# AIM-SE/AC-TSR

Measured on AMD Instinct MI355X. Metric: user-sequences/sec fwd+bwd, AC-SASRec L=50 d=64, 1/2/4/8 MI355X, higher is better.
Workload: dtype f32; 1 GPU; ACSASRec full training step (spatial + adversarial calibrators, BASELINE configs[2]), synthetic 100000-item catalogue, B=512/GPU L=50 d=64 h=2 2 layers inner=256, CE loss, two-pass backward + Adam; global_batch=512, seq_len=50, hidden=64, heads=2, parallelism=dp1, launch=hipGraph replay per step, backward=two walks (reference protocol, trainer.py:672-686)

## Files before the change

ac_tsr_amd/csrc/acattn_bwd.hip:

```cpp
#include <stdlib.h>

#include "acattn_common.h"

int acattn_launch_bwd_general_dh16(const acattn_problem& p, const acattn_bwd_io& io, hipStream_t stream);
int acattn_launch_bwd_general_dh32(const acattn_problem& p, const acattn_bwd_io& io, hipStream_t stream);
int acattn_launch_bwd_general_dh64(const acattn_problem& p, const acattn_bwd_io& io, hipStream_t stream);
int acattn_launch_bwd_general_dh128(const acattn_problem& p, const acattn_bwd_io& io, hipStream_t stream);

int acattn_launch_bwd_fast(const acattn_problem& p, const acattn_bwd_io& io, hipStream_t stream);
int acattn_launch_bwd_stream(const acattn_problem& p, const acattn_bwd_io& io, hipStream_t stream);
int acattn_launch_bwd_onerow(const acattn_problem& p, const acattn_bwd_io& io, bool accumulate, hipStream_t stream);
int acattn_launch_bwd_long(const acattn_problem& p, const acattn_bwd_io& io, hipStream_t stream);

namespace {
thread_local int g_bwd_kernel = ACATTN_BWD_AUTO;
}
int acattn_bwd_kernel_choice(int which) {
  const int old = g_bwd_kernel;
  if (which >= ACATTN_BWD_AUTO && which <= ACATTN_BWD_LONG) g_bwd_kernel = which;
  return old;
}

bool acattn_bwd_onerow_applies(const acattn_problem& p, const acattn_bwd_io& io);

namespace {
bool onerow_split_applies(const acattn_problem& p, const acattn_bwd_io& io) {
  static const bool split = getenv("ACATTN_ONEROW_SPLIT") ? atoi(getenv("ACATTN_ONEROW_SPLIT")) != 0 : true;
  if (!(split && (io.d_attack_mask || io.d_penalty_part) && io.read_rows && io.n_read_rows == 1 && !io.active_qblocks && !io.attack_only && p.L <= 64))
    return false;
  const int dh = p.n_heads > 0 ? p.H / p.n_heads : 0;
  if (dh != 16 && dh != 32 && dh != 64) return false;
  acattn_bwd_io row_io = io;
  row_io.d_attack_mask = nullptr;
  row_io.d_penalty_part = nullptr;
  return acattn_bwd_onerow_applies(p, row_io);
}
}

bool acattn_bwd_gate_summed(const acattn_problem& p, const acattn_bwd_io& io) {
  if (g_bwd_kernel != ACATTN_BWD_AUTO || !io.dgate_logits) return false;
  return acattn_bwd_onerow_applies(p, io) || onerow_split_applies(p, io);
}

bool acattn_bwd_stream_pair_applies(const acattn_problem& p, const acattn_bwd_io& io);
bool acattn_bwd_pair_supported(const acattn_problem& p, const acattn_bwd_io& io) {
  const bool streaming = g_bwd_kernel == ACATTN_BWD_STREAM || (g_bwd_kernel == ACATTN_BWD_AUTO && p.L > 64);
  return streaming && acattn_bwd_stream_pair_applies(p, io);
}

int acattn_launch_bwd(const acattn_problem& p, const acattn_bwd_io& io, hipStream_t stream) {
  if (g_bwd_kernel == ACATTN_BWD_LONG || (g_bwd_kernel == ACATTN_BWD_AUTO && p.L > 208))
    return acattn_launch_bwd_long(p, io, stream);
  if (p.L > 208) {
    acattn_set_error("backward: the pinned kernel is built for L <= 208; L > 208 needs ACATTN_BWD_LONG or ACATTN_BWD_AUTO");
    return -1;
  }
  if ((io.dqa2 || io.dka2 || io.d_ctx_calibrated2 || io.d_penalty_part2) && !acattn_bwd_pair_supported(p, io)) {
    acattn_set_error("attention backward: a second cotangent set was given but this launch cannot evaluate it "
                     "(ask acattn_calibrated_attention_bwd_pair_supported first)");
    return -1;
  }
  if (io.dgate_summed && !acattn_bwd_gate_summed(p, io)) {
    acattn_set_error("attention backward: dgate_summed requested but this launch does not take the one-row form "
                     "(ask acattn_calibrated_attention_bwd_gate_summed first)");
    return -1;
  }
  const int which = g_bwd_kernel;
  if (which == ACATTN_BWD_AUTO) {
    const int rc_one = acattn_launch_bwd_onerow(p, io, false, stream);
    if (rc_one != -100) return rc_one;
    static const bool split = getenv("ACATTN_ONEROW_SPLIT") ? atoi(getenv("ACATTN_ONEROW_SPLIT")) != 0 : true;
    if (split && (io.d_attack_mask || io.d_penalty_part) && io.read_rows && io.n_read_rows == 1 && !io.active_qblocks && !io.attack_only && p.L <= 64) {
      acattn_bwd_io mask_io = io;
      mask_io.d_ctx_attacked = mask_io.d_ctx_calibrated = nullptr;
      mask_io.n_read_rows = 0;
      mask_io.attack_only = 1;
      const int rc_mask = acattn_launch_bwd_fast(p, mask_io, stream);
      if (rc_mask == 0) {
        acattn_bwd_io row_io = io;
        row_io.d_attack_mask = nullptr;
        row_io.d_penalty_part = nullptr;
        const int rc_row = acattn_launch_bwd_onerow(p, row_io, true, stream);
        if (rc_row != -100) return rc_row;
        acattn_set_error("attention backward: the mask-only launch ran but the one-row kernel does not cover this problem (read-row chain not computed)");
        return -1;
      }
      if (rc_mask != -100) return rc_mask;
    }
    if (io.dgate_summed) {
      acattn_set_error("attention backward: dgate_summed was accepted but no one-row form ran");
      return -1;
    }
  }
  static const bool short_stream = getenv("ACATTN_BWD_SHORT_STREAM") && atoi(getenv("ACATTN_BWD_SHORT_STREAM")) != 0;
  const bool short_rows = p.L <= 64 && !short_stream;
  if (which == ACATTN_BWD_AUTO && short_rows) {
    const int rc_fast = acattn_launch_bwd_fast(p, io, stream);
    if (rc_fast != -100) return rc_fast;
  }
  if (which == ACATTN_BWD_AUTO || which == ACATTN_BWD_STREAM) {
    const int rc_stream = acattn_launch_bwd_stream(p, io, stream);
    if (rc_stream != -100) return rc_stream;
  }
  const int rc_fast = acattn_launch_bwd_fast(p, io, stream);
  if (rc_fast != -100) return rc_fast;
  switch (p.H / p.n_heads) {
    case 16: return acattn_launch_bwd_general_dh16(p, io, stream);
    case 32: return acattn_launch_bwd_general_dh32(p, io, stream);
    case 64: return acattn_launch_bwd_general_dh64(p, io, stream);
    case 128: return acattn_launch_bwd_general_dh128(p, io, stream);
  }
  return -1;
}
```

ac_tsr_amd/csrc/acattn_bwd_stream.hip:

```cpp
#include <stdlib.h>

#include <algorithm>

#include "acattn_common.h"

namespace {

constexpr float kLog2e = 1.44269504088896340736f;
constexpr float kLn2 = 0.69314718055994530942f;

__device__ __forceinline__ float ex2(float x) { return __builtin_amdgcn_exp2f(x); }
__device__ __forceinline__ float and_bits(float x, int m) { return __uint_as_float(__float_as_uint(x) & (uint32_t)m); }
__device__ __forceinline__ float hsum(const f4 v) { return (v[0] + v[1]) + (v[2] + v[3]); }
__device__ __forceinline__ float row16_sum(float v) {
  v += __builtin_bit_cast(float, __builtin_amdgcn_update_dpp(0, __builtin_bit_cast(int, v), 0xB1, 0xF, 0xF, false));
  v += __builtin_bit_cast(float, __builtin_amdgcn_update_dpp(0, __builtin_bit_cast(int, v), 0x4E, 0xF, 0xF, false));
  v += __builtin_bit_cast(float, __builtin_amdgcn_update_dpp(0, __builtin_bit_cast(int, v), 0x141, 0xF, 0xF, false));
  v += __builtin_bit_cast(float, __builtin_amdgcn_update_dpp(0, __builtin_bit_cast(int, v), 0x140, 0xF, 0xF, false));
  return v;
}

#ifndef ACATTN_BWD_ONE_WAVE_DH
#define ACATTN_BWD_ONE_WAVE_DH 64
#endif
// ... 842 lines not shown
  } while (0)
#else
#define OR_STAMP(k)
#endif

template <int DH, bool ACC, bool SLICED>
__global__ void __launch_bounds__(64) acattn_bwd_onerow_kernel(const acattn_problem P, const acattn_bwd_io IO) {
#ifdef ACATTN_ONEROW_STAMPS
  unsigned long long cyc_[8] = {}, last_ = 0;
#endif
  OR_STAMP(-1);
  constexpr int D4 = DH / 4;
  __shared__ __attribute__((aligned(16))) float vec[8][DH];
  __shared__ __attribute__((aligned(16))) float col[4][256];
  const int L = P.L, H = P.H, nh = P.n_heads;
  const int nT = (L + 15) >> 4;
  const bool causal = P.causal != 0;
  int b, h;
  decode_block(blockIdx.x, P.B, nh, b, h);
  const int lane = threadIdx.x;
  const size_t rowbase = (size_t)b * L, bh = (size_t)b * nh + h;
  const int hoff = h * DH;
  const int i = min(max((int)IO.read_rows[b], 0), L - 1);
  const KeyFlags F = load_key_flags(P.key_valid, rowbase, L, nT, lane);
  const Consts K = make_consts(P, DH);

  for (int d = lane; d < DH; d += 64) {
    const size_t o = (rowbase + i) * H + hoff + d;
    vec[0][d] = P.q[o];
    vec[1][d] = P.qa[o];
    vec[2][d] = IO.d_ctx_attacked ? IO.d_ctx_attacked[o] : 0.f;
    vec[3][d] = IO.d_ctx_calibrated ? IO.d_ctx_calibrated[o] : 0.f;
    vec[4][d] = P.w_order[DH + d] * -kLog2e;
    vec[5][d] = P.w_dist[DH + d];
    vec[6][d] = P.w_order[d];
    vec[7][d] = P.w_dist[d];
  }
  __syncthreads();
  OR_STAMP(0);
  RowScalars R;
  {
    float ao = 0.f, adv = 0.f;
#pragma unroll
    for (int d = 0; d < DH; ++d) {
      ao += vec[0][d] * vec[6][d];
      adv += vec[0][d] * vec[7][d];
    }
    R.ao2 = -kLog2e * (ao + P.b_order[0]);
    R.ad = adv + P.b_dist[0];
  }
  const bool dead = causal ? F.first_valid > i : !F.any_valid;
  {
    const float sh = dead ? ACATTN_MASK_FILL : 0.f;
    const float* sp = IO.row_stats + (bh * L + i) * ACATTN_NSTAT;
    R.lx2 = (sp[0] - sh) * kLog2e;
    R.ly2 = (sp[1] - sh) * kLog2e;
    R.lu2 = (sp[2] - sh) * kLog2e;
    R.lv2 = (sp[3] - sh) * kLog2e;
    R.lw2 = (sp[4] - sh) * kLog2e;
  }
  R.i = i;
  R.rng_row = (uint32_t)(bh * L + i);
  const bool order_select = !causal || dead;

  constexpr bool sliced = SLICED;
  constexpr int N4 = SLICED ? D4 / 4 : D4;
  const int kgrp = sliced ? (lane & 15) : lane;
  const int slice = sliced ? (lane >> 4) : 0;
  const int d_lo = slice * N4;
  const float lead = slice == 0 ? 1.0f : 0.0f;
  const int t = kgrp >> 2, g = kgrp & 3, j0 = 4 * kgrp;
  f4 aS = {0.f, 0.f, 0.f, 0.f}, aM = aS, aP = aS, aW = aS, co4 = aS, cd4 = aS;
  if constexpr (SLICED) {
#pragma unroll
    for (int r = 0; r < 4; ++r) {
      const size_t o = (rowbase + min(j0 + r, L - 1)) * H + hoff;
#pragma unroll
      for (int k4 = 0; k4 < N4; ++k4) {
        const int d4 = d_lo + k4;
        const f4 kv = *(const f4*)(P.k + o + 4 * d4), kav = *(const f4*)(P.ka + o + 4 * d4), vv = *(const f4*)(P.v + o + 4 * d4);
        const f4 q4 = *(const f4*)(&vec[0][4 * d4]), qa4 = *(const f4*)(&vec[1][4 * d4]);
        const f4 ga4 = *(const f4*)(&vec[2][4 * d4]), gc4 = *(const f4*)(&vec[3][4 * d4]);
        const f4 wo4 = *(const f4*)(&vec[4][4 * d4]), wd4 = *(const f4*)(&vec[5][4 * d4]);
        aS[r] += hsum(kv * q4);
        aM[r] += hsum(kav * qa4);
        aP[r] += hsum(vv * ga4);
        aW[r] += hsum(vv * gc4);
        co4[r] += hsum(kv * wo4);
        cd4[r] += hsum(kv * wd4);
      }
    }
  } else {
    size_t o4[4];
#pragma unroll
    for (int r = 0; r < 4; ++r) o4[r] = (rowbase + min(j0 + r, L - 1)) * H + hoff;
#pragma unroll 2
    for (int k4 = 0; k4 < N4; ++k4) {
      const f4 q4 = *(const f4*)(&vec[0][4 * k4]), qa4 = *(const f4*)(&vec[1][4 * k4]);
      const f4 ga4 = *(const f4*)(&vec[2][4 * k4]), gc4 = *(const f4*)(&vec[3][4 * k4]);
      const f4 wo4 = *(const f4*)(&vec[4][4 * k4]), wd4 = *(const f4*)(&vec[5][4 * k4]);
      f4 kv[4], kav[4], vv[4];
#pragma unroll
      for (int r = 0; r < 4; ++r) {
        kv[r] = *(const f4*)(P.k + o4[r] + 4 * k4);
        kav[r] = *(const f4*)(P.ka + o4[r] + 4 * k4);
        vv[r] = *(const f4*)(P.v + o4[r] + 4 * k4);
      }
#pragma unroll
      for (int r = 0; r < 4; ++r) {
        aS[r] += hsum(kv[r] * q4);
        aM[r] += hsum(kav[r] * qa4);
        aP[r] += hsum(vv[r] * ga4);
        aW[r] += hsum(vv[r] * gc4);
        co4[r] += hsum(kv[r] * wo4);
        cd4[r] += hsum(kv[r] * wd4);
      }
    }
    __builtin_amdgcn_sched_barrier(0);
  }
  if (sliced) {
#pragma unroll
    for (int r = 0; r < 4; ++r) {
      aS[r] = quad_sum(aS[r]);
      aM[r] = quad_sum(aM[r]);
      aP[r] = quad_sum(aP[r]);
      aW[r] = quad_sum(aW[r]);
      co4[r] = quad_sum(co4[r]);
      cd4[r] = quad_sum(cd4[r]);
    }
  }
  OR_STAMP(1);
  const f4 gl = load_seg(P.gate_logits + (rowbase + i) * L, j0, L, true);
  uint32_t eb4, ab4;
  tile_bits(F, t, g, i, L, causal, true, dead, eb4, ab4);
  if (j0 >= 16 * nT) eb4 = 0u;
  Tile T;
  tile_elementwise(R, K, aS, aM, aP, aW, co4, cd4, gl, t, g, eb4, ab4, order_select, T);

  const float da = wave_sum(lead * hsum(T.Ap * T.dAp)), dc = wave_sum(lead * hsum(T.Aw * T.dAw));
  const f4 dw = T.Aw * (T.dAw - dc);
  const f4 dac = (1.0f - T.gt) * dw;
  const float r1 = wave_sum(lead * hsum(T.Ac * dac));
  const f4 du = T.Ap * (T.dAp - da), dv = T.Ac * (dac - r1);
  f4 dP = T.gt * dw + dv * T.ex1 + du * T.M;
  f4 dM = du * (T.P - T.nz) - dv * (T.P * T.ex1);
#pragma unroll
  for (int r = 0; r < 4; ++r) {
    dP[r] = keep_and(dP[r] * K.keep_scale, T.ka, r);
    dM[r] = keep_and(dM[r] * K.keep_scale, T.km, r);
  }
  const float sP = wave_sum(lead * hsum(T.Pt * dP)), sM = wave_sum(lead * hsum(T.Mt * dM));
  f4 dS, dSa, dgl, d_o, d_d;
  float dsc;
  tile_backward(T, K, da, dc, r1, sP, sM, f4{0.f, 0.f, 0.f, 0.f}, i, j0, dS, dSa, dgl, d_o, d_d, dsc);
  const float da_o = wave_sum(lead * hsum(d_o)), da_d = wave_sum(lead * hsum(d_d)), dsc_sum = wave_sum(lead * dsc);
  if (slice == 0) {
    *(f4*)(&col[0][j0]) = dS;
    *(f4*)(&col[1][j0]) = dSa;
    *(f4*)(&col[2][j0]) = d_o;
    *(f4*)(&col[3][j0]) = d_d;
  }

  OR_STAMP(2);
  if constexpr (SLICED) {
#pragma unroll
    for (int r = 0; r < 4; ++r) {
      const int j = j0 + r;
      if (j < L) {
        const size_t o = (rowbase + j) * H + hoff;
#pragma unroll
        for (int k4 = 0; k4 < N4; ++k4) {
          const int d4 = d_lo + k4;
          const f4 q4 = *(const f4*)(&vec[0][4 * d4]), qa4 = *(const f4*)(&vec[1][4 * d4]);
          const f4 ga4 = *(const f4*)(&vec[2][4 * d4]), gc4 = *(const f4*)(&vec[3][4 * d4]);
          const f4 wo_hi = *(const f4*)(P.w_order + DH + 4 * d4), wd_hi = *(const f4*)(P.w_dist + DH + 4 * d4);
          *(f4*)(IO.dk + o + 4 * d4) = q4 * dS[r] + wo_hi * d_o[r] + wd_hi * d_d[r];
          if (ACC)
            *(f4*)(IO.dka + o + 4 * d4) += qa4 * dSa[r];
          else
            *(f4*)(IO.dka + o + 4 * d4) = qa4 * dSa[r];
          *(f4*)(IO.dv + o + 4 * d4) = ga4 * T.Ap[r] + gc4 * T.Aw[r];
        }
      }
    }
  } else {
#pragma unroll 2
    for (int k4 = 0; k4 < N4; ++k4) {
      const f4 q4 = *(const f4*)(&vec[0][4 * k4]), qa4 = *(const f4*)(&vec[1][4 * k4]);
      const f4 ga4 = *(const f4*)(&vec[2][4 * k4]), gc4 = *(const f4*)(&vec[3][4 * k4]);
      const f4 wo_hi = *(const f4*)(P.w_order + DH + 4 * k4), wd_hi = *(const f4*)(P.w_dist + DH + 4 * k4);
#pragma unroll
      for (int r = 0; r < 4; ++r) {
        const int j = j0 + r;
        if (j < L) {
          const size_t o = (rowbase + j) * H + hoff;
          *(f4*)(IO.dk + o + 4 * k4) = q4 * dS[r] + wo_hi * d_o[r] + wd_hi * d_d[r];
          if (ACC)
            *(f4*)(IO.dka + o + 4 * k4) += qa4 * dSa[r];
          else
            *(f4*)(IO.dka + o + 4 * k4) = qa4 * dSa[r];
          *(f4*)(IO.dv + o + 4 * k4) = ga4 * T.Ap[r] + gc4 * T.Aw[r];
        }
      }
    }
    __builtin_amdgcn_sched_barrier(0);
  }
  OR_STAMP(3);
  if (IO.dgate_logits && IO.dgate_summed) {
    if (slice == 0) {
      float* grow = IO.dgate_logits + ((size_t)b * L + i) * L;
#pragma unroll
      for (int r = 0; r < 4; ++r)
        if (j0 + r < L) atomicAdd(grow + j0 + r, dgl[r]);
    }
  } else if (IO.dgate_logits) {
    float* gbase = IO.dgate_logits + bh * (size_t)L * L;
    for (int row = 0; row < L; ++row) {
      if (row == i) continue;
      for (int j = lane; j < L; j += 64) gbase[(size_t)row * L + j] = 0.f;
    }
    if (slice == 0) store_seg(gbase + (size_t)i * L, j0, L, true, dgl);
  }
  __syncthreads();
  OR_STAMP(4);

  const int stride_w = IO.part_stride ? IO.part_stride : 2 * DH, stride_s = IO.part_stride ? IO.part_stride : 4;
  constexpr int PARTS = DH <= 32 ? 64 / DH : 1;
  constexpr int NCH = DH > 64 ? DH / 64 : 1;
#pragma unroll 1
  for (int ch = 0; ch < NCH; ++ch) {
    const int d = (DH > 64 ? lane : lane % DH) + 64 * ch, part = DH > 64 ? 0 : lane / DH;
    float sq = 0.f, sqa = 0.f, so = 0.f, sd = 0.f;
    constexpr int UJ = 8;
    for (int jb = part; jb < L; jb += PARTS * UJ) {
      float kv[UJ], kav[UJ];
#pragma unroll
      for (int u = 0; u < UJ; ++u) {
        const int j = min(jb + u * PARTS, L - 1);
        const size_t o = (rowbase + j) * H + hoff + d;
        kv[u] = P.k[o];
        kav[u] = P.ka[o];
      }
#pragma unroll
      for (int u = 0; u < UJ; ++u) {
        const int j = jb + u * PARTS;
        const float w = j < L ? 1.0f : 0.0f;
        const int jc = min(j, L - 1);
        sq += w * col[0][jc] * kv[u];
        sqa += w * col[1][jc] * kav[u];
        so += w * col[2][jc] * kv[u];
        sd += w * col[3][jc] * kv[u];
      }
    }
#pragma unroll
    for (int off = DH; off < 64; off <<= 1) {
      sq += __shfl_xor(sq, off);
      sqa += __shfl_xor(sqa, off);
      so += __shfl_xor(so, off);
      sd += __shfl_xor(sd, off);
    }
    if (ch == 0) {
      constexpr int LPR = DH / 4, RPI = 64 / LPR;
      const f4 z4 = {0.f, 0.f, 0.f, 0.f};
      for (int row = lane / LPR; row < L; row += RPI) {
        if (row == i) continue;
        const size_t o = (rowbase + row) * H + hoff + 4 * (lane % LPR);
        *(f4*)(IO.dq + o) = z4;
        if (!ACC) *(f4*)(IO.dqa + o) = z4;
      }
    }
    if (part == 0) {
      const size_t o = (rowbase + i) * H + hoff + d;
      IO.dq[o] = sq + da_o * vec[6][d] + da_d * vec[7][d];
      if (ACC) IO.dqa[o] += sqa;
      else IO.dqa[o] = sqa;
    }
    if (part != 0) continue;
    IO.dw_order_part[bh * stride_w + d] = da_o * vec[0][d];
    IO.dw_dist_part[bh * stride_w + d] = da_d * vec[0][d];
    IO.dw_order_part[bh * stride_w + DH + d] = so;
    IO.dw_dist_part[bh * stride_w + DH + d] = sd;
  }
  if (lane == 0) {
    float* sm = IO.dsmall_part + bh * stride_s;
    sm[0] = da_o;
    sm[1] = da_d;
    sm[2] = dsc_sum;
    sm[3] = 0.f;
  }
  OR_STAMP(5);
#ifdef ACATTN_ONEROW_STAMPS
  if (lane == 0 && blockIdx.x < 2048)
    for (int k = 0; k < 8; ++k) g_onerow_stamps[blockIdx.x * 8 + k] = cyc_[k];
#endif
}

#ifdef ACATTN_ONEROW_STAMPS
extern "C" int acattn_debug_onerow_stamps(unsigned long long* host, int n_words) {
  return (int)hipMemcpyFromSymbol(host, HIP_SYMBOL(g_onerow_stamps), (size_t)n_words * 8);
}
#endif

template <int DH>
int launch_onerow(const acattn_problem& p, const acattn_bwd_io& io, bool accumulate, hipStream_t stream) {
  const dim3 grid(p.B * p.n_heads), block(64);
  if (io.dgate_logits && io.dgate_summed) {
    const int rc = acattn_launch_zero(io.dgate_logits, (size_t)p.B * p.L * p.L, stream);
    if (rc) return rc;
  }
  if (p.L <= 64) {
    if (accumulate)
      hipLaunchKernelGGL((acattn_bwd_onerow_kernel<DH, true, true>), grid, block, 0, stream, p, io);
    else
      hipLaunchKernelGGL((acattn_bwd_onerow_kernel<DH, false, true>), grid, block, 0, stream, p, io);
  } else if (accumulate) {
    hipLaunchKernelGGL((acattn_bwd_onerow_kernel<DH, true, false>), grid, block, 0, stream, p, io);
  } else {
    hipLaunchKernelGGL((acattn_bwd_onerow_kernel<DH, false, false>), grid, block, 0, stream, p, io);
  }
  return (int)hipGetLastError();
}

template <int DH>
int launch_stream(const acattn_problem& p, const acattn_bwd_io& io, float* ws, hipStream_t stream) {
  const int nT = (p.L + 15) / 16, dh = DH;
  const size_t rows = (size_t)p.B * p.n_heads;
  if (!io.attack_only) {
    int rc = 0;
    auto zero = [&](float* ptr, size_t n) { if (!rc) rc = acattn_launch_zero(ptr, n, stream); };
    if (io.part_stride) {
      float* lo = std::min(io.dw_order_part, std::min(io.dw_dist_part, io.dsmall_part));
      zero(lo, rows * io.part_stride);
    } else {
      zero(io.dw_order_part, rows * 2 * dh);
      zero(io.dw_dist_part, rows * 2 * dh);
      zero(io.dsmall_part, rows * 4);
    }
    if (rc) return rc;
  }
  const dim3 grid(p.B * p.n_heads * nT), block(64);
  static const bool no_dca_form = getenv("ACATTN_BWD_DCA_ALWAYS") ? atoi(getenv("ACATTN_BWD_DCA_ALWAYS")) == 0 : true;
  if (io.d_ctx_attacked || !no_dca_form) {
    hipLaunchKernelGGL((acattn_bwd_row_kernel<DH, true>), grid, block, 0, stream, p, io, ws);
    hipLaunchKernelGGL((acattn_bwd_key_kernel<DH, true>), grid, block, 0, stream, p, io, (const float*)ws);
  } else if (io.dqa2) {
    hipLaunchKernelGGL((acattn_bwd_row_kernel<DH, false, true>), grid, block, 0, stream, p, io, ws);
    hipLaunchKernelGGL((acattn_bwd_key_kernel<DH, false, true>), grid, block, 0, stream, p, io, (const float*)ws);
  } else {
    hipLaunchKernelGGL((acattn_bwd_row_kernel<DH, false>), grid, block, 0, stream, p, io, ws);
    hipLaunchKernelGGL((acattn_bwd_key_kernel<DH, false>), grid, block, 0, stream, p, io, (const float*)ws);
  }
  return (int)hipGetLastError();
}

}

int64_t acattn_bwd_stream_ws_bytes(const acattn_problem& p) { return (int64_t)p.B * p.n_heads * p.L * NSC * sizeof(float); }

bool acattn_bwd_onerow_applies(const acattn_problem& p, const acattn_bwd_io& io) {
  static const bool enabled = getenv("ACATTN_ONEROW") ? atoi(getenv("ACATTN_ONEROW")) != 0 : true;
  const int dh = p.n_heads > 0 ? p.H / p.n_heads : 0;
  return enabled && io.read_rows && io.n_read_rows == 1 && !io.active_qblocks && !io.d_attack_mask && !io.d_penalty_part && !io.attack_only &&
         p.L <= 208 && (int64_t)p.B * p.n_heads * p.L * p.L < (1LL << 30) && (int64_t)p.B * p.L * p.H < (1LL << 30) &&
         p.mask_mode == ACATTN_MASK_STRUCTURED && p.rng_mode == ACATTN_RNG_COUNTER && p.w_order && p.w_dist &&
         p.adversarial && p.combine_option == ACATTN_COMBINE_GATE && p.two_level && (dh == 16 || dh == 32 || dh == 64 || dh == 128);
}

int acattn_launch_bwd_onerow(const acattn_problem& p, const acattn_bwd_io& io, bool accumulate, hipStream_t stream) {
  if (!acattn_bwd_onerow_applies(p, io)) return -100;
  switch (p.H / p.n_heads) {
    case 16: return launch_onerow<16>(p, io, accumulate, stream);
    case 32: return launch_onerow<32>(p, io, accumulate, stream);
    case 64: return launch_onerow<64>(p, io, accumulate, stream);
    case 128: return launch_onerow<128>(p, io, accumulate, stream);
  }
  return -100;
}

bool acattn_bwd_stream_pair_applies(const acattn_problem& p, const acattn_bwd_io& io) {
  const int dh = p.n_heads > 0 ? p.H / p.n_heads : 0;
  return io.workspace && p.L <= 208 && (int64_t)p.B * p.n_heads * p.L * p.L < (1LL << 30) && (int64_t)p.B * p.L * p.H < (1LL << 30) &&
         p.mask_mode == ACATTN_MASK_STRUCTURED && p.rng_mode == ACATTN_RNG_COUNTER && p.w_order && p.w_dist && p.adversarial &&
         p.combine_option == ACATTN_COMBINE_GATE && p.two_level && (dh == 16 || dh == 32 || dh == 64) && !io.d_ctx_attacked &&
         !io.attack_only && !io.read_rows && !io.active_qblocks && io.dqa2 && io.dka2 &&
         (io.d_ctx_calibrated2 || io.d_penalty_part2);
}

int acattn_launch_bwd_stream(const acattn_problem& p, const acattn_bwd_io& io, hipStream_t stream) {
  const bool ok = io.workspace && p.L <= 208 && (int64_t)p.B * p.n_heads * p.L * p.L < (1LL << 30) &&
                  (int64_t)p.B * p.L * p.H < (1LL << 30) && p.mask_mode == ACATTN_MASK_STRUCTURED &&
                  p.rng_mode == ACATTN_RNG_COUNTER && p.w_order && p.w_dist && p.adversarial &&
                  p.combine_option == ACATTN_COMBINE_GATE && p.two_level;
  if (!ok) return -100;
  float* ws = (float*)io.workspace;
  switch (p.H / p.n_heads) {
    case 16: return launch_stream<16>(p, io, ws, stream);
    case 32: return launch_stream<32>(p, io, ws, stream);
    case 64: return launch_stream<64>(p, io, ws, stream);
    case 128: return launch_stream<128>(p, io, ws, stream);
  }
  return -100;
}
```

Measured before the change: 531,100 user-sequences/sec.

## Add dedicated attack-only attention backward kernel and fold gate zeroing into it

Adds a specialised backward kernel for the attack-mask/penalty-only pass. It runs one block per (batch, head) with one wave per 16-row query block, and builds dK from LDS slot partials without atomics. The same kernel also zeroes the summed gate-logit gradient buffer, so the one-row kernel can skip its separate zero-fill launch. This is meant to replace the generic fast kernel on this path and remove one launch. In exchange it adds sizeable LDS per block and a fallback turn-taking path when there are too few slots.

Result: faster. 537,200 user-sequences/sec, median of 6 (+1.2%).

```diff
diff --git a/ac_tsr_amd/csrc/acattn_bwd.hip b/ac_tsr_amd/csrc/acattn_bwd.hip
--- a/ac_tsr_amd/csrc/acattn_bwd.hip
+++ b/ac_tsr_amd/csrc/acattn_bwd.hip
@@ -9,7 +9,8 @@
 
 int acattn_launch_bwd_fast(const acattn_problem& p, const acattn_bwd_io& io, hipStream_t stream);
 int acattn_launch_bwd_stream(const acattn_problem& p, const acattn_bwd_io& io, hipStream_t stream);
-int acattn_launch_bwd_onerow(const acattn_problem& p, const acattn_bwd_io& io, bool accumulate, hipStream_t stream);
+int acattn_launch_bwd_attack(const acattn_problem& p, const acattn_bwd_io& io, hipStream_t stream, float* gate_zero = nullptr);
+int acattn_launch_bwd_onerow(const acattn_problem& p, const acattn_bwd_io& io, bool accumulate, hipStream_t stream, bool gate_zeroed = false);
 int acattn_launch_bwd_long(const acattn_problem& p, const acattn_bwd_io& io, hipStream_t stream);
 
 namespace {
@@ -24,6 +25,10 @@
 bool acattn_bwd_onerow_applies(const acattn_problem& p, const acattn_bwd_io& io);
 
 namespace {
+bool attack_kernel_enabled() {
+  static const bool on = getenv("ACATTN_BWD_ATTACK") ? atoi(getenv("ACATTN_BWD_ATTACK")) != 0 : true;
+  return on;
+}
 bool onerow_split_applies(const acattn_problem& p, const acattn_bwd_io& io) {
   static const bool split = getenv("ACATTN_ONEROW_SPLIT") ? atoi(getenv("ACATTN_ONEROW_SPLIT")) != 0 : true;
   if (!(split && (io.d_attack_mask || io.d_penalty_part) && io.read_rows && io.n_read_rows == 1 && !io.active_qblocks && !io.attack_only && p.L <= 64))
@@ -75,12 +80,15 @@
       mask_io.d_ctx_attacked = mask_io.d_ctx_calibrated = nullptr;
       mask_io.n_read_rows = 0;
       mask_io.attack_only = 1;
-      const int rc_mask = acattn_launch_bwd_fast(p, mask_io, stream);
+      float* gate_zero = io.dgate_logits && io.dgate_summed ? io.dgate_logits : nullptr;
+      int rc_mask = attack_kernel_enabled() ? acattn_launch_bwd_attack(p, mask_io, stream, gate_zero) : -100;
+      const bool gate_zeroed = rc_mask == 0 && gate_zero;
+      if (rc_mask == -100) rc_mask = acattn_launch_bwd_fast(p, mask_io, stream);
       if (rc_mask == 0) {
         acattn_bwd_io row_io = io;
         row_io.d_attack_mask = nullptr;
         row_io.d_penalty_part = nullptr;
-        const int rc_row = acattn_launch_bwd_onerow(p, row_io, true, stream);
+        const int rc_row = acattn_launch_bwd_onerow(p, row_io, true, stream, gate_zeroed);
         if (rc_row != -100) return rc_row;
         acattn_set_error("attention backward: the mask-only launch ran but the one-row kernel does not cover this problem (read-row chain not computed)");
         return -1;
@@ -95,6 +103,10 @@
   static const bool short_stream = getenv("ACATTN_BWD_SHORT_STREAM") && atoi(getenv("ACATTN_BWD_SHORT_STREAM")) != 0;
   const bool short_rows = p.L <= 64 && !short_stream;
   if (which == ACATTN_BWD_AUTO && short_rows) {
+    if (io.attack_only && attack_kernel_enabled()) {
+      const int rc_attack = acattn_launch_bwd_attack(p, io, stream);
+      if (rc_attack != -100) return rc_attack;
+    }
     const int rc_fast = acattn_launch_bwd_fast(p, io, stream);
     if (rc_fast != -100) return rc_fast;
   }
diff --git a/ac_tsr_amd/csrc/acattn_bwd_attack.hip b/ac_tsr_amd/csrc/acattn_bwd_attack.hip
--- /dev/null
+++ b/ac_tsr_amd/csrc/acattn_bwd_attack.hip
@@ -0,0 +1,308 @@
+#include <stdlib.h>
+
+#include <type_traits>
+
+#include "acattn_common.h"
+
+namespace {
+
+constexpr float kLog2e = 1.44269504088896340736f;
+
+__device__ __forceinline__ float ex2(float x) { return __builtin_amdgcn_exp2f(x); }
+__device__ __forceinline__ float hsum(const f4 v) { return (v[0] + v[1]) + (v[2] + v[3]); }
+
+constexpr int TS = 20;
+
+template <int DH>
+__global__ void __launch_bounds__(256, 4) acattn_bwd_attack_kernel(const acattn_problem P, const acattn_bwd_io IO, float* gate_zero,
+                                                                    const int n_slots) {
+  constexpr int KS = DH / 4;
+  constexpr int DT = DH / 16;
+  constexpr int VS = DH + 4;
+  constexpr int SLOT = 16 * VS;
+
+  const int L = P.L, H = P.H, nh = P.n_heads;
+  const int nT = (L + 15) >> 4;
+  const int LP = nT * 16;
+  int b, h;
+  decode_block(blockIdx.x, P.B, nh, b, h);
+  const int lane = threadIdx.x & 63;
+  const int wave = __builtin_amdgcn_readfirstlane(threadIdx.x >> 6);
+  const int c = lane & 15, g = lane >> 4;
+  const size_t rowbase = (size_t)b * L;
+  const int hoff = h * DH;
+  const size_t bh = (size_t)b * nh + h;
+
+  extern __shared__ __attribute__((aligned(16))) float smem[];
+  float* Kas = smem;
+  float* s_km = Kas + LP * VS;
+  float* scr_all = s_km + LP;
+  float* slots = scr_all + nT * 16 * TS;
+  float* scr = scr_all + wave * 16 * TS;
+
+  const int qb = wave, i0 = qb * 16, i = i0 + c;
+  const bool row_ok = i < L;
+  float qaf[KS];
+  {
+    const size_t off = (rowbase + (row_ok ? i : 0)) * H + hoff + KS * g;
+#pragma unroll
+    for (int s4 = 0; s4 < KS / 4; ++s4) {
+      f4 ta = {0.f, 0.f, 0.f, 0.f};
+      if (row_ok) ta = *(const f4*)(P.qa + off + 4 * s4);
+#pragma unroll
+      for (int e = 0; e < 4; ++e) qaf[4 * s4 + e] = ta[e];
+    }
+  }
+  const float lse_y2 = row_ok ? IO.row_stats[(bh * L + i) * ACATTN_NSTAT + 1] * kLog2e : 0.f;
+  float qac[4][DT];
+#pragma unroll
+  for (int s = 0; s < 4; ++s) {
+    const int row = i0 + 4 * g + s;
+    const float* p = P.qa + (rowbase + min(row, L - 1)) * H + hoff + c;
+#pragma unroll
+    for (int dt = 0; dt < DT; ++dt) qac[s][dt] = row < L ? p[16 * dt] : 0.f;
+  }
+
+  constexpr int KV_IT = DH / 16;
+  f4 r_ka[KV_IT];
+#pragma unroll
+  for (int it = 0; it < KV_IT; ++it) {
+    const int idx = threadIdx.x + it * blockDim.x;
+    const int row = idx / (DH / 4), c4 = idx - row * (DH / 4);
+    r_ka[it] = f4{0.f, 0.f, 0.f, 0.f};
+    if (row < L) r_ka[it] = *(const f4*)(P.ka + (rowbase + row) * H + hoff + 4 * c4);
+  }
+  const uint8_t r_valid = (threadIdx.x < L) ? P.key_valid[rowbase + threadIdx.x] : (uint8_t)0;
+  if (gate_zero && h == 0) {
+    float* zp = gate_zero + rowbase * L;
+    const int n = L * L;
+    for (int j = 4 * threadIdx.x; j < n; j += 4 * blockDim.x) {
+      if (j + 3 < n) {
+        *(f4u*)(zp + j) = f4{0.f, 0.f, 0.f, 0.f};
+      } else {
+        for (int r = 0; j + r < n; ++r) zp[j + r] = 0.f;
+      }
+    }
+  }
+#pragma unroll
+  for (int it = 0; it < KV_IT; ++it) {
+    const int idx = threadIdx.x + it * blockDim.x;
+    const int row = idx / (DH / 4), c4 = idx - row * (DH / 4);
+    *(f4*)(Kas + row * VS + 4 * c4) = r_ka[it];
+  }
+  if (threadIdx.x < LP) {
+    const int j = threadIdx.x;
+    float km = ACATTN_NEG_INF;
+    if (j < L) km = r_valid ? 0.f : ACATTN_MASK_FILL * kLog2e;
+    s_km[j] = km;
+  }
+  const uint64_t seed_eff = P.seed + (P.seed_device ? *P.seed_device : 0ull);
+  const RngKey rkey = rng_key(seed_eff);
+  __syncthreads();
+
+  const unsigned long long valid_keys = __ballot(lane < L && s_km[lane] == 0.f);
+  const int first_valid = valid_keys ? __ffsll((long long)valid_keys) - 1 : L;
+  const bool causal = P.causal != 0;
+  const int nt_valid = valid_keys ? ((63 - __clzll((long long)valid_keys)) >> 4) + 1 : nT;
+  auto tiles_of_block = [&](int q) {
+    const bool rows_see_a_key = causal ? first_valid <= 16 * q : valid_keys != 0;
+    return rows_see_a_key ? min(causal ? min(nT, q + 1) : nT, nt_valid) : nT;
+  };
+  int nts[4], base[4], total = 0;
+#pragma unroll
+  for (int q = 0; q < 4; ++q) {
+    nts[q] = q < nT ? tiles_of_block(q) : 0;
+    base[q] = total;
+    total += nts[q];
+  }
+  const int nt = tiles_of_block(qb);
+  const int my_base = qb == 0 ? base[0] : qb == 1 ? base[1] : qb == 2 ? base[2] : base[3];
+  const bool in_turns = total > n_slots;
+
+  const float inv_sqrt = 1.0f / sqrtf((float)DH);
+  const float scale2 = inv_sqrt * kLog2e;
+  const bool has_drop = P.p_drop > 0.f;
+  const float keep_scale = has_drop ? 1.0f / (1.0f - P.p_drop) : 1.0f;
+  const uint32_t prow = ((uint32_t)bh * L + (row_ok ? i : 0)) * (uint32_t)L;
+  const float dpen2 = IO.d_penalty_part ? 2.0f * IO.d_penalty_part[(size_t)bh * nT + qb] : 0.f;
+  const uint32_t rng_row = (uint32_t)(bh * L + i);
+  const float okf = row_ok ? 1.0f : 0.0f;
+
+  auto mask4 = [&](int t) -> f4 {
+    const f4 km4 = *(const f4*)(s_km + 16 * t + 4 * g);
+    if (causal && (16 * t + 15 > i0)) {
+      const int dq = (c - 4 * g) + 16 * (qb - t);
+      f4 m;
+#pragma unroll
+      for (int r = 0; r < 4; ++r) m[r] = (dq < r) ? fminf(km4[r], ACATTN_MASK_FILL * kLog2e) : km4[r];
+      return m;
+    }
+    return km4;
+  };
+  auto load_seg = [&](const float* rowp, int t) -> f4 {
+    const int j0 = 16 * t + 4 * g;
+    f4 v = {0.f, 0.f, 0.f, 0.f};
+    if (row_ok && j0 < L) {
+      const float* p = rowp + j0;
+      if (j0 + 3 < L) {
+        v = *(const f4u*)p;
+      } else {
+#pragma unroll
+        for (int r = 0; r < 4; ++r)
+          if (j0 + r < L) v[r] = p[r];
+      }
+    }
+    return v;
+  };
+
+  auto body = [&](auto ntb_c) {
+    constexpr int NTB = decltype(ntb_c)::value;
+
+    f4 tM[NTB], dMa[NTB];
+#pragma unroll
+    for (int t = 0; t < NTB; ++t) tM[t] = f4{0.f, 0.f, 0.f, 0.f};
+#pragma unroll
+    for (int s4 = 0; s4 < KS / 4; ++s4) {
+#pragma unroll
+      for (int t = 0; t < NTB; ++t) {
+        const f4 x4 = *(const f4*)(Kas + (16 * t + c) * VS + KS * g + 4 * s4);
+#pragma unroll
+        for (int e = 0; e < 4; ++e) tM[t] = mfma16(x4[e], qaf[4 * s4 + e], tM[t]);
+      }
+    }
+#pragma unroll
+    for (int t = 0; t < NTB; ++t) {
+      const f4 y = tM[t] * scale2 + mask4(t);
+#pragma unroll
+      for (int r = 0; r < 4; ++r) tM[t][r] = ex2(y[r] - lse_y2) * okf;
+    }
+
+    float r2 = 0.f;
+#pragma unroll
+    for (int t = 0; t < NTB; ++t) {
+      uint32_t keep = 0xFu;
+      if (has_drop)
+        keep = P.p_drop == 0.5f ? rng_keep_mask_half(rkey, rng_row, (uint32_t)(4 * t + g))
+                                : rng_group(rkey, rng_row, (uint32_t)(4 * t + g), P.p_drop).keep_mask;
+      const f4 sm = keep_scale4(keep, keep_scale);
+      dMa[t] = f4{0.f, 0.f, 0.f, 0.f};
+      if (IO.d_attack_mask) dMa[t] = load_seg(IO.d_attack_mask + prow, t);
+      if (IO.d_penalty_part) dMa[t] += (tM[t] * sm - 1.0f) * dpen2;
+      dMa[t] *= sm;
+      r2 += hsum(tM[t] * dMa[t]);
+    }
+    r2 = quad_sum(r2);
+#pragma unroll
+    for (int t = 0; t < NTB; ++t) dMa[t] = (tM[t] * (dMa[t] - r2)) * inv_sqrt;
+
+    {
+      f4 oqa[DT];
+#pragma unroll
+      for (int dt = 0; dt < DT; ++dt) oqa[dt] = f4{0.f, 0.f, 0.f, 0.f};
+#pragma unroll
+      for (int t = 0; t < NTB; ++t)
+#pragma unroll
+        for (int r = 0; r < 4; ++r) {
+          const float* kap = Kas + (16 * t + 4 * g + r) * VS + c;
+#pragma unroll
+          for (int dt = 0; dt < DT; ++dt) oqa[dt] = mfma16(kap[16 * dt], dMa[t][r], oqa[dt]);
+        }
+      if (row_ok) {
+        const uint32_t off = ((uint32_t)rowbase + i) * H + hoff + 4 * g;
+#pragma unroll
+        for (int dt = 0; dt < DT; ++dt) *(f4*)(IO.dqa + off + 16 * dt) = oqa[dt];
+      }
+    }
+
+    auto key_side = [&](auto sink) {
+#pragma unroll
+      for (int t = 0; t < NTB; ++t) {
+        asm volatile("s_waitcnt lgkmcnt(0)" ::: "memory");
+        *(f4*)(scr + c * TS + 4 * g) = dMa[t];
+        asm volatile("s_waitcnt lgkmcnt(0)" ::: "memory");
+        f4 o[DT];
+#pragma unroll
+        for (int dt = 0; dt < DT; ++dt) o[dt] = f4{0.f, 0.f, 0.f, 0.f};
+#pragma unroll
+        for (int s = 0; s < 4; ++s) {
+          const float b_sa = scr[(4 * g + s) * TS + c];
+#pragma unroll
+          for (int dt = 0; dt < DT; ++dt) o[dt] = mfma16(qac[s][dt], b_sa, o[dt]);
+        }
+        sink(t, o);
+      }
+    };
+    if (!in_turns) {
+      key_side([&](int t, const f4 (&o)[DT]) {
+        float* sl = slots + (my_base + t) * SLOT + c * VS + 4 * g;
+#pragma unroll
+        for (int dt = 0; dt < DT; ++dt) *(f4*)(sl + 16 * dt) = o[dt];
+      });
+      __syncthreads();
+    } else {
+      for (int j = lane; j < SLOT; j += 64) slots[wave * SLOT + j] = 0.f;
+      __syncthreads();
+      for (int q = 0; q < nT; ++q) {
+        if (q == qb)
+          key_side([&](int t, const f4 (&o)[DT]) {
+            float* sl = slots + t * SLOT + c * VS + 4 * g;
+#pragma unroll
+            for (int dt = 0; dt < DT; ++dt) *(f4*)(sl + 16 * dt) += o[dt];
+          });
+        __syncthreads();
+      }
+    }
+  };
+  switch (nt) {
+    case 1: body(std::integral_constant<int, 1>{}); break;
+    case 2: body(std::integral_constant<int, 2>{}); break;
+    case 3: body(std::integral_constant<int, 3>{}); break;
+    default: body(std::integral_constant<int, 4>{}); break;
+  }
+
+  for (int idx = threadIdx.x; idx < L * (DH / 4); idx += blockDim.x) {
+    const int row = idx / (DH / 4), c4 = idx - row * (DH / 4);
+    const int t = row >> 4, in = (row & 15) * VS + 4 * c4;
+    f4 sum = {0.f, 0.f, 0.f, 0.f};
+    if (in_turns) {
+      sum = *(const f4*)(slots + t * SLOT + in);
+    } else {
+#pragma unroll
+      for (int q = 0; q < 4; ++q)
+        if (nts[q] > t) sum += *(const f4*)(slots + (base[q] + t) * SLOT + in);
+    }
+    *(f4*)(IO.dka + (rowbase + row) * H + hoff + 4 * c4) = sum;
+  }
+}
+
+template <int DH>
+int launch_attack(const acattn_problem& p, const acattn_bwd_io& io, float* gate_zero, hipStream_t stream) {
+  const int nT = (p.L + 15) / 16, LP = nT * 16;
+  const int n_slots = p.causal ? nT * (nT + 1) / 2 : nT * nT;
+  const size_t lds = (size_t)(LP * (DH + 4) + LP + nT * 16 * TS + n_slots * 16 * (DH + 4)) * sizeof(float);
+  auto kern = acattn_bwd_attack_kernel<DH>;
+  if (lds > 64 * 1024) {
+    const hipError_t e = hipFuncSetAttribute((const void*)kern, hipFuncAttributeMaxDynamicSharedMemorySize, (int)lds);
+    if (e != hipSuccess) return (int)e;
+  }
+  hipLaunchKernelGGL(kern, dim3(p.B * p.n_heads), dim3(64 * nT), lds, stream, p, io, gate_zero, n_slots);
+  return (int)hipGetLastError();
+}
+
+}
+
+int acattn_launch_bwd_attack(const acattn_problem& p, const acattn_bwd_io& io, hipStream_t stream, float* gate_zero) {
+  const bool ok = p.L >= 1 && p.L <= 64 && (int64_t)p.B * p.n_heads * p.L * p.L < (1LL << 30) && (int64_t)p.B * p.L * p.H < (1LL << 30) &&
+                  p.mask_mode == ACATTN_MASK_STRUCTURED && p.rng_mode == ACATTN_RNG_COUNTER && p.w_order && p.w_dist &&
+                  p.adversarial && p.combine_option == ACATTN_COMBINE_GATE && p.two_level && io.attack_only &&
+                  (io.d_attack_mask || io.d_penalty_part) && !io.d_ctx_attacked && !io.d_ctx_calibrated &&
+                  !(io.read_rows && io.n_read_rows > 0) && !io.active_qblocks && !io.dqa2 && !io.dka2 && io.dqa && io.dka &&
+                  io.row_stats;
+  if (!ok) return -100;
+  switch (p.H / p.n_heads) {
+    case 16: return launch_attack<16>(p, io, gate_zero, stream);
+    case 32: return launch_attack<32>(p, io, gate_zero, stream);
+    case 64: return launch_attack<64>(p, io, gate_zero, stream);
+  }
+  return -100;
+}
diff --git a/ac_tsr_amd/csrc/acattn_bwd_stream.hip b/ac_tsr_amd/csrc/acattn_bwd_stream.hip
--- a/ac_tsr_amd/csrc/acattn_bwd_stream.hip
+++ b/ac_tsr_amd/csrc/acattn_bwd_stream.hip
@@ -1168,9 +1168,9 @@
 #endif
 
 template <int DH>
-int launch_onerow(const acattn_problem& p, const acattn_bwd_io& io, bool accumulate, hipStream_t stream) {
+int launch_onerow(const acattn_problem& p, const acattn_bwd_io& io, bool accumulate, bool gate_zeroed, hipStream_t stream) {
   const dim3 grid(p.B * p.n_heads), block(64);
-  if (io.dgate_logits && io.dgate_summed) {
+  if (io.dgate_logits && io.dgate_summed && !gate_zeroed) {
     const int rc = acattn_launch_zero(io.dgate_logits, (size_t)p.B * p.L * p.L, stream);
     if (rc) return rc;
   }
@@ -1232,13 +1232,13 @@
          p.adversarial && p.combine_option == ACATTN_COMBINE_GATE && p.two_level && (dh == 16 || dh == 32 || dh == 64 || dh == 128);
 }
 
-int acattn_launch_bwd_onerow(const acattn_problem& p, const acattn_bwd_io& io, bool accumulate, hipStream_t stream) {
+int acattn_launch_bwd_onerow(const acattn_problem& p, const acattn_bwd_io& io, bool accumulate, hipStream_t stream, bool gate_zeroed) {
   if (!acattn_bwd_onerow_applies(p, io)) return -100;
   switch (p.H / p.n_heads) {
-    case 16: return launch_onerow<16>(p, io, accumulate, stream);
-    case 32: return launch_onerow<32>(p, io, accumulate, stream);
-    case 64: return launch_onerow<64>(p, io, accumulate, stream);
-    case 128: return launch_onerow<128>(p, io, accumulate, stream);
+    case 16: return launch_onerow<16>(p, io, accumulate, gate_zeroed, stream);
+    case 32: return launch_onerow<32>(p, io, accumulate, gate_zeroed, stream);
+    case 64: return launch_onerow<64>(p, io, accumulate, gate_zeroed, stream);
+    case 128: return launch_onerow<128>(p, io, accumulate, gate_zeroed, stream);
   }
   return -100;
 }
```
